# naturerobots/mesh_navigation

Hardware: AMD Instinct MI355X
Metric: plans/sec (Dijkstra makePlan device path incl. computeVectorMap, 1M-vertex mesh) (higher is better)
Workload: dtype f32

## Files before the change

mesh_navigation_amd/csrc/mnav_options.h:

```cpp
#pragma once

#define MNAV_OPTION_LIST(X)                                                                                                              \
  X(verbose)                                                              \
  X(trace)                                                                                       \
  X(no_graph)             \
  X(debug_chunk)                                                                            \
  X(dijkstra_engine)                                 \
  X(blocks_per_plan)                                                                                 \
  X(tile_blocks)                                                                                    \
  X(cvp_wide)                                        \
  X(wide_waves)                                                                                      \
  X(cvp_groups)                          \
  X(max_steps) X(max_wall_s)                                                                                                             \
  X(cvp_verify)                                                                     \
  X(key_walk_max) X(descend_walk_max)                                                               \
  X(tile_size)                                                                                   \
  X(lazy_paths)                                                                                      \
  X(tile_band) X(rounds_band_mult)                                                                                                       \
  X(tb_tile)                                                       \
  X(tb_no_prefill) X(tb_band_mult) X(tb_waves_per_cu)                                                                                    \
  X(tb_kernel)            \
  X(async_wg_per_cu) X(async_wg_per_plan) X(async_max_s)                                                                                 \
  X(async_band_mult)                              \
  X(async_max_batch)                                           \
  X(async_ring_cap)             \
  X(nbhd_lds_cap)         \
  X(replan_log_cap)                                          \
  X(replan_fresh_below)   \
  X(replan_each_fresh_share)  \
  X(replan_repair_engine)  \
  X(replan_warm_min_plans)  \
  X(fleet_scratch_mb)     \
  X(dispatch_max_mb)      \
  X(dispatch_max_rounds)  \
  X(dispatch_tail_bidders)

struct Options {
#define X(name) double name = NAN;
  MNAV_OPTION_LIST(X)
#undef X
  struct Desc { const char* name; double Options::*field; };
  static const Desc* table(size_t* n)
  {
    static const Desc t[] = {
#define X(name) { #name, &Options::name },
      MNAV_OPTION_LIST(X)
#undef X
    };
    *n = sizeof(t) / sizeof(t[0]);
    return t;
  }
  double* find(const char* name)
  {
    size_t n; const Desc* t = table(&n);
    for (size_t i = 0; i < n; ++i) if (!strcmp(t[i].name, name)) return &(this->*t[i].field);
    return nullptr;
  }
  void from_environment()
  {
    size_t n; const Desc* t = table(&n);
    for (size_t i = 0; i < n; ++i) {
      std::string var = "MNAV_";
      for (const char* c = t[i].name; *c; ++c) var += (char)toupper((unsigned char)*c);
      const char* e = getenv(var.c_str());
      if (!e || !*e) continue;
      double v = atof(e);
      if (!strcmp(t[i].name, "dijkstra_engine")) {
        v = !strcmp(e, "tiled") ? 0 : !strcmp(e, "band") ? 1 : !strcmp(e, "tile_batch") ? 5 : !strcmp(e, "async") ? 6
          : (e[0] >= '0' && e[0] <= '9') ? atof(e) : 3;
      }
      this->*t[i].field = v;
    }
  }
};
static inline bool opt_set(double v) { return v == v; }
static inline uint32_t opt_u32(double v, uint32_t dflt) { return v == v ? (uint32_t)(v < 0.0 ? 0.0 : v) : dflt; }
static inline bool opt_on(double v) { return v == v && v != 0.0; }
```

mesh_navigation_amd/csrc/mnav_tb.h:

```cpp
#pragma once

#include "mnav_tb_build.h"

namespace {

namespace tb {

#define MNAV_CONST __attribute__((address_space(4)))
typedef uint32_t u32x16 __attribute__((ext_vector_type(16)));
typedef const MNAV_CONST u32x16* cblk8_t;
typedef __attribute__((address_space(3))) uint32_t* lds_u32_t;
enum { kTwSoff = 0, kTwSl = 1, kTwNv = 2, kTwNh = 3, kTwSweepOff = 4, kTwSweepChunks = 5, kTwPreOff = 6, kTwPreChunks = 7,
       kTwPostOff = 8, kTwPostChunks = 9, kTwExpOff = 10, kTwExpN = 11 };
static_assert(offsetof(TbTile, exp_n) == 4 * kTwExpN && offsetof(TbTile, sweep_off) == 4 * kTwSweepOff, "TbTile layout");

struct Ctl {
  uint32_t n_cand[2];
  uint32_t n_items, next_item;
  uint32_t err;
  uint32_t iters;
  unsigned long long acts;
  unsigned long long sweeps;
  unsigned long long items;
  unsigned long long wakes;
};

struct Args {
  const TbTile* tiles; const uint32_t* stream; const TbExp* exps;
  float* D; uint32_t* pend; uint32_t NP, ntiles;
  uint16_t* bucket; uint32_t* bcnt; uint2* items; Ctl* ctl;
  uint32_t* marr[2];
  uint32_t* mcarry;
  float* thr; float* bnd;
  const uint32_t* seed; const uint32_t* target;
  const uint2* vaddr; const uint32_t* vert_tile;
  double offset; float band;
  uint8_t* pflag; uint32_t nblk;
  unsigned long long* wstat; uint32_t wstat_slots;
  uint32_t item_plans;
};

__device__ __forceinline__ size_t slot_addr(const uint2 va, uint32_t NP, uint32_t p)
{
  return (size_t)va.x * NP + (size_t)p * (va.y >> 8) + (va.y & 255u);
}

__device__ __forceinline__ uint32_t ldsr(uint32_t off) { return *(lds_u32_t)(uintptr_t)off; }
__device__ __forceinline__ void ldsw(uint32_t off, uint32_t v) { *(lds_u32_t)(uintptr_t)off = v; }
typedef __attribute__((address_space(3))) u32x4* lds_u32x4_t;
__device__ __forceinline__ u32x4 ldsr4(uint32_t off) { return *(lds_u32x4_t)(uintptr_t)off; }

__device__ __forceinline__ uint32_t rfl(uint32_t x) { return (uint32_t)__builtin_amdgcn_readfirstlane((int)x); }

}

__global__ __launch_bounds__(kBlock) void k_tb_weights(size_t n, const uint32_t* __restrict__ wsrc, const Nbr* __restrict__ nbr, uint32_t* __restrict__ stream)
{
  const size_t stride = (size_t)gridDim.x * kBlock;
  for (size_t i = (size_t)blockIdx.x * kBlock + threadIdx.x; i < n; i += stride) {
    const uint32_t s = wsrc[i];
    if (s != kNone) stream[i] = f2u(nbr[s].w);
  }
}

__global__ __launch_bounds__(kBlock) void k_tb_fill(u32x4* __restrict__ p, size_t n16, uint32_t v)
{
  const size_t stride = (size_t)gridDim.x * kBlock;
  const u32x4 x = { v, v, v, v };
  for (size_t i = (size_t)blockIdx.x * kBlock + threadIdx.x; i < n16; i += stride) __builtin_nontemporal_store(x, p + i);
}

__global__ __launch_bounds__(kBlock) void k_tb_seed(tb::Args A)
{
  const uint32_t p = blockIdx.x * kBlock + threadIdx.x;
  if (p >= A.NP) return;
  const uint32_t s = A.seed[p];
  const uint2 va = A.vaddr[s];
  A.D[tb::slot_addr(va, A.NP, p)] = 0.0f;
  const uint32_t t = A.vert_tile[s];
  const TbTile W = A.tiles[t];
  const uint32_t row = (va.y & 255u) * 256u;
  for (uint32_t k = 0; k < W.exp_n; ++k) {
    const TbExp e = A.exps[W.exp_off + k];
    if (e.u == row) A.D[(size_t)e.soff * A.NP + (size_t)p * e.sl + e.off] = 0.0f;
  }
  A.pend[(size_t)t * A.NP + p] = 0u;
  A.pflag[(size_t)t * A.nblk + (p >> 6)] = 1;
  A.marr[0][p] = 0u;
  A.ctl->n_cand[0] = 1u;
}

constexpr uint32_t kTbMinCopies = 64;
__global__ __launch_bounds__(kBlock) void k_tb_plan(tb::Args A, int par)
{
  const uint32_t p = blockIdx.x * kBlock + threadIdx.x;
  if (p == 0) { A.ctl->n_cand[par ^ 1] = 0u; A.ctl->next_item = 0u; A.ctl->n_items = 0u; A.ctl->iters += 1u; }
  if (p >= A.NP) return;
  uint32_t mb = A.marr[par][p];
  A.marr[par ^ 1][p] = kTbInfBits;
  {
    uint32_t x[kTbMinCopies];
#pragma unroll
    for (uint32_t c = 0; c < kTbMinCopies; ++c) x[c] = A.mcarry[(size_t)c * A.NP + p];
#pragma unroll
    for (uint32_t c = 0; c < kTbMinCopies; ++c) {
      mb = min(mb, x[c]);
      if (x[c] != kTbInfBits) A.mcarry[(size_t)c * A.NP + p] = kTbInfBits;
    }
  }
  const float m = u2f(mb);
  const float dt = A.D[tb::slot_addr(A.vaddr[A.target[p]], A.NP, p)];
  const float bound = (float)((double)dt + fmax(A.offset, 0.0));
  const bool done = !(m < inf_f()) || m > bound;
  float thr = m + A.band;
  if (!(thr > m)) thr = next_up(m);
  A.thr[p] = done ? 0.0f : thr;
  A.bnd[p] = bound;
}

constexpr uint32_t kTbStatSlots = 16384;
constexpr uint32_t kTbSchedTiles = kBlock / 64;
#ifndef MNAV_TB_SCHED_DEPTH
#define MNAV_TB_SCHED_DEPTH 4
#endif
constexpr uint32_t kTbSchedDepth = MNAV_TB_SCHED_DEPTH;
__global__ __launch_bounds__(kBlock) void k_tb_sched(tb::Args A, int par)
{
  const uint32_t lane = threadIdx.x & 63u;
  const uint32_t t = tb::rfl(blockIdx.x * kTbSchedTiles + (threadIdx.x >> 6));
  if (t >= A.ntiles) return;
  const uint32_t nblk = A.nblk, NP = A.NP;
  MNAV_GLOBAL uint8_t* const g_flag = as_global(A.pflag) + (size_t)t * nblk;
  auto flags = [&](uint32_t c) { const uint32_t i = c * 64u + lane; return i < nblk ? (uint32_t)g_flag[i] : 0u; };
  const uint32_t f0 = flags(0u), f1 = flags(1u);
  unsigned long long m = __ballot(f0 != 0u), m_next = __ballot(f1 != 0u);
  uint32_t c = 0;
  auto next_block = [&]() -> uint32_t {
    while (m == 0ull) {
      if ((c + 1u) * 64u >= nblk) return kNone;
      ++c; m = m_next; m_next = __ballot(flags(c + 1u) != 0u);
    }
    const uint32_t b = c * 64u + (uint32_t)__builtin_ctzll(m);
    m &= m - 1ull;
    return b;
  };
  const uint32_t b_first = next_block();
  if (b_first == kNone) return;
  MNAV_GLOBAL const float* const g_thr = as_global(A.thr);
  MNAV_GLOBAL const float* const g_bnd = as_global(A.bnd);
  MNAV_GLOBAL uint32_t* const g_pend = as_global(A.pend) + (size_t)t * NP;
  MNAV_GLOBAL uint16_t* const g_bucket = as_global(A.bucket) + (size_t)t * NP;
  MNAV_GLOBAL uint32_t* const g_min = as_global(A.mcarry) + (size_t)(t % kTbMinCopies) * NP;
  struct Row { uint32_t p, pb, pm; float thr, bnd; bool live; };
  auto fetch = [&](uint32_t b) {
    Row r;
    const uint32_t p = (b != kNone ? b : 0u) * 64u + lane;
    r.live = b != kNone && p < NP;
    r.p = r.live ? p : 0u;
    r.pb = g_pend[r.p]; r.thr = g_thr[r.p]; r.bnd = g_bnd[r.p]; r.pm = g_min[r.p];
    return r;
  };
  const unsigned long long below = (1ull << lane) - 1ull;
  uint32_t count = 0;
  bool carried = false;
  constexpr int K = (int)kTbSchedDepth;
  uint32_t b_cur[K];
  Row cur[K];
  b_cur[0] = b_first;
#pragma unroll
  for (int k = 1; k < K; ++k) b_cur[k] = next_block();
#pragma unroll
  for (int k = 0; k < K; ++k) cur[k] = fetch(b_cur[k]);
  for (;;) {
    uint32_t b_next[K];
    Row nxt[K];
#pragma unroll
    for (int k = 0; k < K; ++k) b_next[k] = next_block();
#pragma unroll
    for (int k = 0; k < K; ++k) nxt[k] = fetch(b_next[k]);
    __builtin_amdgcn_sched_barrier(0);
#pragma unroll
    for (int k = 0; k < K; ++k)
      asm volatile("" :: "v"(cur[k].pb), "v"(cur[k].thr), "v"(cur[k].bnd), "v"(cur[k].pm));
#pragma unroll
    for (int k = 0; k < K; ++k) {
      if (b_cur[k] == kNone) break;
      const uint32_t p = cur[k].p, pb = cur[k].pb;
      bool ready = false, keep = false;
      if (cur[k].live && pb != kTbInfBits) {
        const float pv = u2f(pb);
        if (pv > cur[k].bnd) g_pend[p] = kTbInfBits;
        else if (pv < cur[k].thr) { g_pend[p] = kTbInfBits; ready = true; }
        else {
          keep = true;
          if (pb < cur[k].pm) atomicMin((uint32_t*)(g_min + p), pb);
        }
      }
      const bool any_keep = __any(keep);
      carried |= any_keep;
      if (!any_keep && lane == 0u) g_flag[b_cur[k]] = 0;
      const unsigned long long rm = __ballot(ready);
      if (ready) g_bucket[count + (uint32_t)__popcll(rm & below)] = (uint16_t)p;
      count += (uint32_t)__popcll(rm);
    }
    if (b_next[0] == kNone) break;
#pragma unroll
    for (int k = 0; k < K; ++k) { cur[k] = nxt[k]; b_cur[k] = b_next[k]; }
  }
  if (lane == 0u) {
    if (count) A.bcnt[t] = count;
    if (carried) A.ctl->n_cand[par ^ 1] = 1u;
  }
}

constexpr uint32_t kTbItemPlans = 16;
__global__ __launch_bounds__(kBlock) void k_tb_items(tb::Args A)
{
  const uint32_t t = blockIdx.x * kBlock + threadIdx.x;
  const int lane = threadIdx.x & 63;
  const uint32_t gran = A.item_plans;
  uint32_t c = 0;
  if (t < A.ntiles) { c = A.bcnt[t]; if (c) A.bcnt[t] = 0u; }
  const uint32_t k = (c + gran - 1u) / gran;
  uint32_t incl = k;
#pragma unroll
  for (int o = 1; o < 64; o <<= 1) { const uint32_t x = __shfl_up(incl, o); if (lane >= o) incl += x; }
  __shared__ uint32_t s_wave[kBlock / 64], s_base;
  const int wave = threadIdx.x >> 6;
  if (lane == 63) s_wave[wave] = incl;
  __syncthreads();
  if (threadIdx.x == 0) {
    uint32_t tot = 0;
#pragma unroll
    for (int w = 0; w < kBlock / 64; ++w) { const uint32_t x = s_wave[w]; s_wave[w] = tot; tot += x; }
    s_base = tot ? atomicAdd(&A.ctl->n_items, tot) : 0u;
  }
  __syncthreads();
  const uint32_t base = s_base + s_wave[wave] + incl - k;
  for (uint32_t q = 0; q < k; ++q) A.items[base + q] = make_uint2(t, (q * gran) | (min(gran, c - q * gran) << 16));
}

__global__ __launch_bounds__(1024) void k_tb_stats(tb::Args A)
{
  __shared__ unsigned long long s_part[16][4];
  unsigned long long acc[4] = { 0ull, 0ull, 0ull, 0ull };
  for (uint32_t w = threadIdx.x; w < A.wstat_slots; w += 1024u)
#pragma unroll
    for (int k = 0; k < 4; ++k) acc[k] += A.wstat[4u * w + k];
#pragma unroll
  for (int k = 0; k < 4; ++k)
#pragma unroll
    for (int o = 32; o > 0; o >>= 1) acc[k] += __shfl_xor(acc[k], o);
  if ((threadIdx.x & 63u) == 0u)
#pragma unroll
    for (int k = 0; k < 4; ++k) s_part[threadIdx.x >> 6][k] = acc[k];
  __syncthreads();
  if (threadIdx.x == 0) {
    unsigned long long t[4] = { 0ull, 0ull, 0ull, 0ull };
    for (int w = 0; w < 16; ++w)
      for (int k = 0; k < 4; ++k) t[k] += s_part[w][k];
    A.ctl->items = t[0]; A.ctl->acts = t[1]; A.ctl->sweeps = t[2]; A.ctl->wakes = t[3];
  }
}

struct TbBlk { uint32_t ya, raw, v[7]; };

#ifdef MNAV_TB_TIMING
__device__ unsigned long long g_tb_timing[8];
#define TB_STAMP(k) do { const unsigned long long now_ = __builtin_readcyclecounter(); tt[k] += now_ - t_last; t_last = now_; } while (0)
#else
#define TB_STAMP(k) do { } while (0)
#endif

constexpr uint32_t kTbQStride = 272;

namespace tb {
__device__ __forceinline__ void ldsw4(uint32_t off, u32x4 v) { *(lds_u32x4_t)(uintptr_t)off = v; }
__device__ __forceinline__ uint32_t wmax4(uint32_t x)
{
  x = max(x, (uint32_t)__shfl_xor((int)x, 16));
  x = max(x, (uint32_t)__shfl_xor((int)x, 32));
  return rfl(x);
}
struct QStream {
  MNAV_GLOBAL const u32x4* st;
  uint32_t last, wr, c; u32x4 c1;
  __device__ __forceinline__ void begin_at(MNAV_GLOBAL const u32x4* first, uint32_t nch, uint32_t stage_q, uint32_t l16)
  {
    st = first + l16;
    last = nch ? nch - 1u : 0u; wr = stage_q + 16u * l16; c = 0;
    ldsw4(wr, st[0]);
    c1 = st[(size_t)min(1u, last) * 16u];
  }
  __device__ __forceinline__ void begin(MNAV_GLOBAL const uint32_t* stream, uint32_t chunk_off, uint32_t nch, uint32_t stage_q, uint32_t l16)
  {
    begin_at((MNAV_GLOBAL const u32x4*)(stream + (size_t)chunk_off * kTbChunk), nch, stage_q, l16);
  }
  __device__ __forceinline__ void advance()
// ... 387 lines not shown
    const uint32_t beg = row_ptr[v], end = row_ptr[v + 1];
    for (uint32_t i = beg + lane; i < end; i += kWave) {
      const Nbr nb = nbr[i];
      const float du = A.D[tb::slot_addr(A.vaddr[nb.u], A.NP, p)];
      if (!expanded_source(gcut, du, nb.u)) continue;
      const float sm = du + nb.w;
      if (sm < best_s || (sm == best_s && sm < inf_f() && (du < best_du || (du == best_du && nb.u < best_u)))) { best_s = sm; best_du = du; best_u = nb.u; }
    }
#pragma unroll
    for (int o = 1; o < kWave; o <<= 1) {
      const float os = __shfl_xor(best_s, o), odu = __shfl_xor(best_du, o);
      const uint32_t ou = __shfl_xor(best_u, o);
      if (os < best_s || (os == best_s && os < inf_f() && (odu < best_du || (odu == best_du && ou < best_u)))) { best_s = os; best_du = odu; best_u = ou; }
    }
    if (!(best_s < inf_f())) best_u = v;
  }
  if (lane == 0) {
    float x = 0.f, y = 0.f, z = 0.f;
    if (best_u != v) {
      x = xyz[3 * (size_t)best_u] - xyz[3 * (size_t)v];
      y = xyz[3 * (size_t)best_u + 1] - xyz[3 * (size_t)v + 1];
      z = xyz[3 * (size_t)best_u + 2] - xyz[3 * (size_t)v + 2];
      const float len = sqrtf(x * x + y * y + z * z);
      x = x / len; y = y / len; z = z / len;
    }
    out[3 * blockIdx.x] = x; out[3 * blockIdx.x + 1] = y; out[3 * blockIdx.x + 2] = z;
  }
}

__global__ __launch_bounds__(kBlock) void k_tb_count(tb::Args A, uint32_t T, PlanResult* __restrict__ res)
{
  const uint32_t t = blockIdx.x;
  const int lane = threadIdx.x & 63, wid = threadIdx.x >> 6;
  const TbTile W = A.tiles[t];
  for (uint32_t p = blockIdx.y * (kBlock / 64) + wid; p < A.NP; p += gridDim.y * (kBlock / 64)) {
    const float dt = A.D[tb::slot_addr(A.vaddr[A.target[p]], A.NP, p)];
    const float goal_dist = goal_cut(dt, A.offset, A.target[p]).cut;
    const float* sl = A.D + ((size_t)W.soff * A.NP + (size_t)p * W.sl);
    uint32_t c = 0;
    for (uint32_t i = lane; i < W.nv; i += 64) { const float d = sl[i]; c += (d < inf_f() && d <= goal_dist) ? 1u : 0u; }
    c = wave_sum(c);
    if (lane == 0 && c) atomicAdd(&res[p].settled, (unsigned long long)c);
  }
}

__global__ __launch_bounds__(kBlock) void k_tb_popped(tb::Args A, uint32_t p, uint32_t V, float* __restrict__ out)
{
  const float dt = A.D[tb::slot_addr(A.vaddr[A.target[p]], A.NP, p)];
  const float goal_dist = goal_cut(dt, A.offset, A.target[p]).cut;
  const uint32_t stride = gridDim.x * kBlock;
  for (uint32_t v = blockIdx.x * kBlock + threadIdx.x; v < V; v += stride) {
    const float d = A.D[tb::slot_addr(A.vaddr[v], A.NP, p)];
    out[v] = (d <= goal_dist) ? d : inf_f();
  }
}

__global__ __launch_bounds__(kBlock) void k_popped(const float* __restrict__ dist, uint32_t target, double offset, uint32_t V, float* __restrict__ out)
{
  const float dt = dist[target];
  const float goal_dist = goal_cut(dt, offset, target).cut;
  const uint32_t stride = gridDim.x * kBlock;
  for (uint32_t v = blockIdx.x * kBlock + threadIdx.x; v < V; v += stride) { const float d = dist[v]; out[v] = (d <= goal_dist) ? d : inf_f(); }
}

struct TbTables {
  bool built = false, w_valid = false;
  uint32_t ntiles = 0, max_nh = 0;
  uint64_t S = 0;
  size_t nrec = 0, nexp = 0;
  std::vector<uint32_t> vert_tile;
  DevBuf<uint32_t> d_verts;
  DevBuf<TbTile> d_tiles; DevBuf<uint32_t> d_stream, d_wsrc; DevBuf<TbExp> d_exps;
  DevBuf<uint32_t> d_vstream, d_vwsrc, d_vtile, d_vgroups; DevBuf<TbvExp> d_vexps; size_t nvrec = 0;
  DevBuf<uint2> d_vaddr; DevBuf<uint32_t> d_vert_tile;
  DevBuf<uint16_t> d_fin_src; DevBuf<uint32_t> d_fin_wsrc; DevBuf<float> d_fin_w; DevBuf<TbFinOvf> d_fin_ovf; DevBuf<uint32_t> d_fin_ovf_wsrc; DevBuf<float> d_fin_ovf_w;
  DevBuf<uint32_t> d_ghost_gid, d_fin_order; size_t fin_n = 0, fin_novf = 0; bool fin_w_valid = false; uint32_t max_sl = 0;
};

struct TbBatch {
  uint32_t cap_np = 0;
  DevBuf<float> D; DevBuf<uint32_t> pend; DevBuf<uint32_t> mcarry; DevBuf<uint8_t> pflag; DevBuf<uint16_t> bucket; DevBuf<uint32_t> bcnt; DevBuf<uint2> items;
  DevBuf<tb::Ctl> ctl; PinnedBuf<tb::Ctl> h_ctl;
  DevBuf<unsigned long long> wstat; DevBuf<struct FinRec> d_recs;
  DevBuf<uint32_t> marr[2];
  DevBuf<float> thr, bnd; DevBuf<uint32_t> seed, target;
  GraphExec graph[2]; tb::Args graph_args[2]{};
  DevBuf<float> D2; bool d2_clean = false; uint32_t d2_clean_np = 0, d2_wanted_np = 0;
};

struct TbState : TbTables, TbBatch {
  uint32_t T = 120;
  int kernel = 0;
  uint32_t min_batch = 48;
  float band_mult = 2.0f;
  int iters_per_replay = 16, waves_per_cu = 0;
  Stream fill_stream; Event fill_done, call_done;
  Event warm_ev[4]; float ms_warm = 0.f, ms_warm_fin = 0.f;
  tb::Ctl last{};
  bool count_pending = false;
};

}

#ifdef MNAV_TB_TIMING
extern "C" int mnav_debug_tb_timing(unsigned long long* out)
{
  if (hipMemcpyFromSymbol(out, HIP_SYMBOL(g_tb_timing), sizeof(unsigned long long) * 8) != hipSuccess) return -1;
  unsigned long long z[8] = { 0, 0, 0, 0, 0, 0, 0, 0 };
  return hipMemcpyToSymbol(HIP_SYMBOL(g_tb_timing), z, sizeof(z)) == hipSuccess ? 0 : -1;
}
#endif
```

mesh_navigation_amd/csrc/mnav_tb_host.h:

```cpp
#pragma once

void tb_free_batch(mnav_ctx* ctx)
{
  TbState& S = ctx->tb;
  if (S.fill_stream) (void)hipStreamSynchronize(S.fill_stream);
  static_cast<TbBatch&>(S) = TbBatch{};
  S.count_pending = false; ctx->tb_args_valid = false;
}

void tb_free(mnav_ctx* ctx)
{
  tb_free_batch(ctx);
  static_cast<TbTables&>(ctx->tb) = TbTables{};
}

int tb_build(mnav_ctx* ctx)
{
  TbState& S = ctx->tb;
  if (S.built) return 0;
  if (opt_set(ctx->opt.tb_tile)) S.T = opt_u32(ctx->opt.tb_tile, S.T);
  if (S.T != 64 && S.T != 96 && S.T != 120 && S.T != 128) S.T = 120;
  HostTopology t;
  t.V = ctx->V; t.E = ctx->E; t.F = ctx->F;
  t.row_ptr = ctx->h_row_ptr; t.nbr_u = ctx->h_nbr_u;
// ... 19 lines not shown
  HIPCHK(S.d_vaddr.upload(ctx->stream, vaddr.data(), vaddr.size()));
  HIPCHK(S.d_vert_tile.upload(ctx->stream, H.vert_tile.data(), H.vert_tile.size()));
  HIPCHK(S.d_verts.upload(ctx->stream, H.verts.data(), H.verts.size()));
  HIPCHK(S.d_fin_src.upload(ctx->stream, H.fin_src.data(), H.fin_src.size()));
  HIPCHK(S.d_fin_wsrc.upload(ctx->stream, H.fin_wsrc.data(), H.fin_wsrc.size()));
  HIPCHK(S.d_fin_ovf.upload(ctx->stream, H.fin_ovf.data(), H.fin_ovf.size()));
  {
    std::vector<uint32_t> ow(H.fin_ovf.size());
    for (size_t i = 0; i < ow.size(); ++i) ow[i] = H.fin_ovf[i].wsrc;
    HIPCHK(S.d_fin_ovf_wsrc.upload(ctx->stream, ow.data(), ow.size()));
  }
  HIPCHK(S.d_ghost_gid.upload(ctx->stream, H.ghost_gid.data(), H.ghost_gid.size()));
  {
    std::vector<uint32_t> order(H.tiles.size()), key(H.tiles.size(), 0xFFFFFFFFu);
    for (size_t t = 0; t < H.tiles.size(); ++t) {
      order[t] = (uint32_t)t;
      for (uint32_t i = 0; i < H.tiles[t].nv; ++i) key[t] = std::min(key[t], H.verts[H.tiles[t].v0 + i]);
    }
    std::stable_sort(order.begin(), order.end(), [&](uint32_t a, uint32_t b) { return key[a] < key[b]; });
    if (order.empty()) order.push_back(0u);
    HIPCHK(S.d_fin_order.upload(ctx->stream, order.data(), order.size()));
  }
  S.d_fin_w.reset(); S.d_fin_ovf_w.reset();
  S.fin_n = H.fin_src.size(); S.fin_novf = H.fin_ovf.size(); S.fin_w_valid = false; S.max_sl = H.max_sl;
  HIPCHK(S.d_fin_w.alloc(4 * std::max<size_t>(S.fin_n, 1)));
  HIPCHK(S.d_fin_ovf_w.alloc(4 * std::max<size_t>(S.fin_novf, 1)));
  HIPCHK(hipStreamSynchronize(ctx->stream));
  S.nvrec = H.vstream.size();
  S.ntiles = H.ntiles; S.S = H.S; S.nrec = H.stream.size(); S.nexp = H.exps.size(); S.max_nh = H.max_nh;
  S.vert_tile = std::move(H.vert_tile);
  S.built = true; S.w_valid = false;
  if (opt_on(ctx->opt.verbose))
    fprintf(stderr, "[mnav] tile-batch engine: T %u, %u tiles, %.2f slots per vertex, max ghosts %u, %.1f MB of streams + %.1f MB of sweep streams in the V layout\n", S.T, S.ntiles,
            ctx->V ? (double)S.S / ctx->V : 0.0, S.max_nh, (4.0 * S.nrec + 16.0 * S.nexp) / 1e6, 4.0 * S.nvrec / 1e6);
  return 0;
}

int tb_weights(mnav_ctx* ctx)
{
  TbState& S = ctx->tb;
  if (S.w_valid) return 0;
  hipLaunchKernelGGL(k_tb_weights, dim3(4096), dim3(kBlock), 0, ctx->stream, S.nrec, S.d_wsrc, ctx->d_nbr, S.d_stream);
  hipLaunchKernelGGL(k_tb_weights, dim3(4096), dim3(kBlock), 0, ctx->stream, S.nvrec, S.d_vwsrc, ctx->d_nbr, S.d_vstream);
  HIPCHK(hipGetLastError());
  S.w_valid = true; S.fin_w_valid = false;
  return 0;
}

int tb_fin_weights(mnav_ctx* ctx)
{
  TbState& S = ctx->tb;
  if (S.fin_w_valid) return 0;
  hipLaunchKernelGGL(k_tb_fin_weights, dim3(4096), dim3(kBlock), 0, ctx->stream, S.fin_n, S.d_fin_wsrc, ctx->d_nbr, S.d_fin_w);
  if (S.fin_novf) hipLaunchKernelGGL(k_tb_fin_weights, dim3(64), dim3(kBlock), 0, ctx->stream, S.fin_novf, S.d_fin_ovf_wsrc, ctx->d_nbr, S.d_fin_ovf_w);
  HIPCHK(hipGetLastError());
  S.fin_w_valid = true;
  return 0;
}

int tb_ensure_batch(mnav_ctx* ctx, uint32_t np)
{
  TbState& S = ctx->tb;
  if (np <= S.cap_np) return 0;
  tb_free_batch(ctx);
  const size_t nt = S.ntiles ? S.ntiles : 1, pairs = nt * (size_t)np;
  HIPCHK(S.D.alloc(4 * (size_t)S.S * np + 64));
  if (8 * (size_t)S.S * np <= ((size_t)96 << 30) && !opt_on(ctx->opt.tb_no_prefill)) {
    if (S.D2.alloc(4 * (size_t)S.S * np + 64) != hipSuccess) (void)hipGetLastError();
    if (S.D2 && !S.fill_stream) { HIPCHK(hipStreamCreateWithFlags(S.fill_stream.out(), hipStreamNonBlocking)); HIPCHK(hipEventCreateWithFlags(S.fill_done.out(), hipEventDisableTiming)); HIPCHK(hipEventCreateWithFlags(S.call_done.out(), hipEventDisableTiming)); }
  }
  HIPCHK(S.pend.alloc(4 * pairs + 64));
  HIPCHK(S.pflag.alloc(nt * (((size_t)np + 63) / 64) + 64));
  HIPCHK(S.bucket.alloc(2 * pairs + 64));
  HIPCHK(S.bcnt.alloc(4 * nt));
  HIPCHK(S.items.alloc(8 * (nt + pairs / kTbItemPlans + 64)));
  HIPCHK(S.ctl.alloc(sizeof(tb::Ctl)));
  HIPCHK(S.wstat.alloc(32 * (size_t)kTbStatSlots));
  HIPCHK(S.h_ctl.alloc(sizeof(tb::Ctl)));
  for (int k = 0; k < 2; ++k) HIPCHK(S.marr[k].alloc(4 * (size_t)np));
  HIPCHK(S.mcarry.alloc(4 * (size_t)kTbMinCopies * np + 64));
  HIPCHK(S.thr.alloc(4 * (size_t)np)); HIPCHK(S.bnd.alloc(4 * (size_t)np));
  HIPCHK(S.seed.alloc(4 * (size_t)np)); HIPCHK(S.target.alloc(4 * (size_t)np));
  HIPCHK(S.d_recs.alloc(sizeof(FinRec) * (size_t)np));
  S.cap_np = np;
  return 0;
}

int tb_fill(mnav_ctx* ctx, void* p, size_t bytes, uint32_t v)
{
  const size_t n16 = (bytes + 15) / 16;
  uint32_t g = (uint32_t)std::min<size_t>((n16 + kBlock - 1) / kBlock, 256 * 32);
  if (g < 1) g = 1;
  hipLaunchKernelGGL(k_tb_fill, dim3(g), dim3(kBlock), 0, ctx->stream, (u32x4*)p, n16, v);
  HIPCHK(hipGetLastError());
  return 0;
}

int tb_launch_iterations(mnav_ctx* ctx, const tb::Args& A, int count, uint32_t waves)
{
  const uint32_t gp = (A.NP + kBlock - 1) / kBlock;
  for (int j = 0; j < count; ++j) {
    const int par = j & 1;
    hipLaunchKernelGGL(k_tb_plan, dim3(gp), dim3(kBlock), 0, ctx->stream, A, par);
    hipLaunchKernelGGL(k_tb_sched, dim3(std::max((A.ntiles + kTbSchedTiles - 1) / kTbSchedTiles, 1u)), dim3(kBlock), 0, ctx->stream, A, par);
    hipLaunchKernelGGL(k_tb_items, dim3((A.ntiles + kBlock - 1) / kBlock), dim3(kBlock), 0, ctx->stream, A);
    if (ctx->tb.kernel == 1) hipLaunchKernelGGL((k_tbv_solve<120>), dim3(waves), dim3(64), 0, ctx->stream, A, ctx->tb.d_vtile, ctx->tb.d_vstream, ctx->tb.d_vgroups, ctx->tb.d_vexps, par);
    else if (ctx->tb.T == 64) hipLaunchKernelGGL((k_tb_solve_q<64>), dim3(waves), dim3(64), 0, ctx->stream, A, par);
    else if (ctx->tb.T == 96) hipLaunchKernelGGL((k_tb_solve_q<96>), dim3(waves), dim3(64), 0, ctx->stream, A, par);
    else if (ctx->tb.T == 120) hipLaunchKernelGGL((k_tb_solve_q<120>), dim3(waves), dim3(64), 0, ctx->stream, A, par);
    else hipLaunchKernelGGL((k_tb_solve_q<128>), dim3(waves), dim3(64), 0, ctx->stream, A, par);
  }
  hipLaunchKernelGGL(k_tb_stats, dim3(1), dim3(1024), 0, ctx->stream, A);
  HIPCHK(hipGetLastError());
  return 0;
}

int tb_fields(mnav_ctx* ctx, uint32_t n, const std::vector<PlanIn>& in, double offset, const tb::Args& A)
{
  TbState& S = ctx->tb;
  if (ensure_slots(ctx, n, false, false, ctx->want_vec)) return -1;
  if (tb_fin_weights(ctx)) return -1;
  std::vector<Plan> hp(n);
  std::vector<float*> vecs(n);
  for (uint32_t i = 0; i < n; ++i) {
    Slot& s = ctx->slots[i];
    Plan& P = hp[i];
    memset(&P, 0, sizeof(P));
    P.planner = kPlannerDijkstra; P.V = ctx->V;
    P.row_ptr = ctx->d_row_ptr.get(); P.nbr = ctx->d_nbr.get(); P.crn_ptr = ctx->d_crn_ptr.get(); P.crn = ctx->d_crn.get(); P.blocked = ctx->d_blocked.get();
    P.dist = s.dist.get(); P.pred = s.pred.get(); P.cap = ctx->V; P.ctl = s.ctl; P.cnt = s.cnt.get();
    P.offset = offset; P.max_steps = ctx->max_steps;
    for (int k = 0; k < 3; ++k) { P.seed[k] = in[i].seed[k]; P.target[k] = in[i].target[k]; P.seed_d[k] = 0.f; P.seed_expands[k] = 1; P.target_expands[k] = 1; }
    P.seed_face = kNone;
    vecs[i] = s.vecmap;
  }
  HIPCHK(hipMemcpyAsync(ctx->d_plans, hp.data(), sizeof(Plan) * n, hipMemcpyHostToDevice, ctx->stream));
  HIPCHK(hipMemcpyAsync(ctx->d_vecptrs, vecs.data(), sizeof(float*) * n, hipMemcpyHostToDevice, ctx->stream));
  HIPCHK(hipStreamSynchronize(ctx->stream));
  FinTb F{};
  F.src = S.d_fin_src; F.w = S.d_fin_w; F.ovf = S.d_fin_ovf; F.ovf_w = S.d_fin_ovf_w; F.verts = S.d_verts; F.ghost_gid = S.d_ghost_gid; F.order = S.d_fin_order;
  F.xyz = ctx->d_xyz; F.vecmaps = ctx->want_vec ? ctx->d_vecptrs : nullptr;
  F.plans = ctx->d_plans; F.res = ctx->d_res; F.mismatch = ctx->d_mismatch; F.recs = S.d_recs;
  const uint32_t groups = (S.ntiles + kFinWaves - 1u) / kFinWaves;
#ifndef MNAV_FIN_PPW
#define MNAV_FIN_PPW 64u
#endif
  F.plans_per_wave = MNAV_FIN_PPW; F.tiles_per_xcd = (groups + 7u) / 8u; F.max_sl = S.max_sl;
  hipLaunchKernelGGL(k_tb_fin_plans, dim3((n + kBlock - 1) / kBlock), dim3(kBlock), 0, ctx->stream, A, ctx->d_plans, F.vecmaps, S.d_recs);
  const uint32_t npg = (n + F.plans_per_wave - 1u) / F.plans_per_wave;
  const size_t lds = 4 * (size_t)fin_lds_words(S.max_sl, F.vecmaps != nullptr) * kFinWaves;
  const dim3 grid(8u * F.tiles_per_xcd * npg);
  if (S.T == 64) hipLaunchKernelGGL((k_tb_finalize<64>), grid, dim3(64 * kFinWaves), lds, ctx->stream, A, F);
  else if (S.T == 96) hipLaunchKernelGGL((k_tb_finalize<96>), grid, dim3(64 * kFinWaves), lds, ctx->stream, A, F);
  else if (S.T == 120) hipLaunchKernelGGL((k_tb_finalize<120>), grid, dim3(64 * kFinWaves), lds, ctx->stream, A, F);
  else hipLaunchKernelGGL((k_tb_finalize<128>), grid, dim3(64 * kFinWaves), lds, ctx->stream, A, F);
  HIPCHK(hipGetLastError());
  return 0;
}

int tb_clean_other(mnav_ctx* ctx)
{
  TbState& S = ctx->tb;
  if (!S.D2 || !S.fill_stream || S.d2_wanted_np == 0u || S.d2_clean) return 0;
  const uint32_t n = S.d2_wanted_np;
  S.d2_wanted_np = 0u;
  const size_t n16 = (4 * (size_t)S.S * n + 15) / 16;
  const uint32_t g = (uint32_t)std::max<size_t>(std::min<size_t>((n16 + kBlock - 1) / kBlock, 256 * 32), 1);
  HIPCHK(hipEventRecord(S.call_done, ctx->stream));
  HIPCHK(hipStreamWaitEvent(S.fill_stream, S.call_done, 0));
  hipLaunchKernelGGL(k_tb_fill, dim3(g), dim3(kBlock), 0, S.fill_stream, (u32x4*)S.D2.get(), n16, kTbInfBits);
  HIPCHK(hipEventRecord(S.fill_done, S.fill_stream));
  S.d2_clean = true; S.d2_clean_np = n;
  return 0;
}

struct TbWarmIn { const uint32_t* d_level; const float* const* d_dist; ReplanCnt* d_cnt; };

int run_dijkstra_tb(mnav_ctx* ctx, uint32_t n, const std::vector<PlanIn>& in, double offset, const TbWarmIn* warm = nullptr)
{
  TbState& S = ctx->tb;
  if (tb_build(ctx)) return -1;
  if (tb_weights(ctx)) return -1;
  if (n > 65535u) { ctx->err = "tile-batch engine: more than 65535 plans in one batch"; return -1; }
  if (tb_ensure_batch(ctx, n)) return -1;
  if (ensure_plan_tables(ctx, n)) return -1;
  if (ensure_paths(ctx, n)) return -1;
  if (!ctx->d_mismatch) HIPCHK(ctx->d_mismatch.alloc(4));
  std::vector<uint32_t> seeds(n), targets(n);
  for (uint32_t i = 0; i < n; ++i) { seeds[i] = in[i].seed[0]; targets[i] = in[i].target[0]; }
  HIPCHK(hipMemcpyAsync(S.seed, seeds.data(), 4 * (size_t)n, hipMemcpyHostToDevice, ctx->stream));
  HIPCHK(hipMemcpyAsync(S.target, targets.data(), 4 * (size_t)n, hipMemcpyHostToDevice, ctx->stream));
  HIPCHK(hipMemsetAsync(ctx->d_res, 0, sizeof(PlanResult) * n, ctx->stream));
  HIPCHK(hipMemsetAsync(ctx->d_mismatch, 0, 4, ctx->stream));
  tb::Args A{};
  A.tiles = S.d_tiles; A.stream = S.d_stream; A.exps = S.d_exps; A.D = S.D; A.pend = S.pend; A.pflag = S.pflag; A.nblk = (n + 63u) / 64u; A.NP = n; A.ntiles = S.ntiles;
  A.bucket = S.bucket; A.bcnt = S.bcnt; A.items = S.items; A.ctl = S.ctl; A.wstat = S.wstat; A.wstat_slots = kTbStatSlots;
  A.marr[0] = S.marr[0]; A.marr[1] = S.marr[1]; A.mcarry = S.mcarry;
  A.thr = S.thr; A.bnd = S.bnd; A.seed = S.seed; A.target = S.target; A.vaddr = S.d_vaddr; A.vert_tile = S.d_vert_tile;
  A.offset = offset;
  const bool v_fits = S.T == 120 && S.max_nh <= kTbvGhostRows;
  const double density = (double)n / std::sqrt((double)std::max(S.ntiles, 1u));
  S.kernel = (v_fits && density >= 8.0) ? 1 : 0;
  if (opt_set(ctx->opt.tb_kernel)) S.kernel = (opt_u32(ctx->opt.tb_kernel, 0u) == 1u && v_fits) ? 1 : 0;
  A.item_plans = S.kernel == 1 ? 64u : kTbItemPlans;
  {
    const float band_mult = (S.kernel == 1 && density < 40.0) ? 4.0f : S.band_mult;
    float band = (ctx->delta_auto / 3.0f) * std::sqrt((float)S.T) * band_mult;
    if (opt_set(ctx->opt.tb_band_mult)) band = (ctx->delta_auto / 3.0f) * std::sqrt((float)S.T) * (float)ctx->opt.tb_band_mult;
    if (ctx->tile_band_user > 0.f) band = ctx->tile_band_user;
    A.band = band;
  }
  HIPCHK(hipEventRecord(ctx->ev[1], ctx->stream));
  if (!warm) {
    bool prefilled = false;
    if (S.D2 && S.d2_clean && S.d2_clean_np >= n) {
      std::swap(S.D, S.D2); A.D = S.D;
      HIPCHK(hipStreamWaitEvent(ctx->stream, S.fill_done, 0));
      prefilled = true;
    }
    S.d2_clean = false;
    if (!prefilled && tb_fill(ctx, S.D, 4 * (size_t)S.S * n, kTbInfBits)) return -1;
    if (tb_fill(ctx, S.pend, 4 * (size_t)S.ntiles * n, kTbInfBits)) return -1;
  }
  HIPCHK(hipMemsetAsync(S.pflag, 0, (size_t)(S.ntiles ? S.ntiles : 1) * ((n + 63u) / 64u) + 64u, ctx->stream));
  if (tb_fill(ctx, S.marr[0], 4 * (size_t)n, kTbInfBits)) return -1;
  if (tb_fill(ctx, S.marr[1], 4 * (size_t)n, kTbInfBits)) return -1;
  if (tb_fill(ctx, S.mcarry, 4 * (size_t)kTbMinCopies * n, kTbInfBits)) return -1;
  HIPCHK(hipMemsetAsync(S.ctl, 0, sizeof(tb::Ctl), ctx->stream));
  HIPCHK(hipMemsetAsync(S.wstat, 0, 32 * (size_t)kTbStatSlots, ctx->stream));
  HIPCHK(hipMemsetAsync(S.bcnt, 0, 4 * (size_t)(S.ntiles ? S.ntiles : 1), ctx->stream));
  if (warm) {
    if (!S.warm_ev[0]) for (auto& e : S.warm_ev) HIPCHK(hipEventCreate(e.out()));
    HIPCHK(hipMemsetAsync(warm->d_cnt, 0, sizeof(ReplanCnt) * (size_t)n, ctx->stream));
    TbWarm Wm{};
    Wm.level = warm->d_level; Wm.dist = warm->d_dist; Wm.cnt = warm->d_cnt;
    Wm.verts = S.d_verts; Wm.ghost_gid = S.d_ghost_gid; Wm.order = S.d_fin_order; Wm.T = S.T;
    const size_t groups = (size_t)std::max(S.ntiles, 1u) * ((n + 63u) / 64u);
    if (groups >= (1ull << 31)) { ctx->err = "tile-batch engine: warm start beyond 2^31 workgroups"; return -1; }
    HIPCHK(hipEventRecord(S.warm_ev[0], ctx->stream));
    if (S.ntiles) hipLaunchKernelGGL(k_tb_warm, dim3((uint32_t)groups), dim3(kWarmBlock), 0, ctx->stream, A, Wm);
    HIPCHK(hipEventRecord(S.warm_ev[1], ctx->stream));
  } else
  hipLaunchKernelGGL(k_tb_seed, dim3((n + kBlock - 1) / kBlock), dim3(kBlock), 0, ctx->stream, A);
  HIPCHK(hipGetLastError());
  HIPCHK(hipEventRecord(ctx->ev[2], ctx->stream));
  if (!warm || !S.d2_clean) S.d2_wanted_np = S.D2 ? n : 0u;

  int ncu = 256;
  (void)hipDeviceGetAttribute(&ncu, hipDeviceAttributeMultiprocessorCount, ctx->device);
  uint32_t per_cu = (uint32_t)((160u * 1024u) / (S.T * 256u + kTbQStride * 4u));
  if (S.kernel == 1) per_cu = 8u;
  if (opt_set(ctx->opt.tb_waves_per_cu)) S.waves_per_cu = (int)ctx->opt.tb_waves_per_cu;
  if (S.waves_per_cu > 0) per_cu = (uint32_t)S.waves_per_cu;
  const uint32_t waves = std::min(per_cu * (uint32_t)ncu, kTbStatSlots);
  const int chunk = S.iters_per_replay & ~1;
  int gi = 0;
  for (int k = 0; k < 2; ++k) if (S.graph[k] && memcmp(&S.graph_args[k], &A, sizeof(A)) == 0) gi = k + 2;
  if (ctx->use_graph && gi < 2) {
    gi = (S.graph[0] && S.graph_args[0].D != A.D) ? 1 : 0;
    S.graph[gi].reset();
    hipGraph_t g = nullptr;
    HIPCHK(hipStreamBeginCapture(ctx->stream, hipStreamCaptureModeThreadLocal));
    const int rc = tb_launch_iterations(ctx, A, chunk, waves);
    const hipError_t e = hipStreamEndCapture(ctx->stream, &g);
    if (rc != 0 || e != hipSuccess) { ctx->err = "graph capture failed"; return -1; }
    HIPCHK(hipGraphInstantiate(S.graph[gi].out(), g, nullptr, nullptr, 0));
    (void)hipGraphDestroy(g);
    memcpy(&S.graph_args[gi], &A, sizeof(A));
  } else gi -= 2;
  int rc = 0;
  uint32_t iters = 0;
  const auto t_start = std::chrono::steady_clock::now();
  HIPCHK(hipEventRecord(ctx->evc[0], ctx->stream));
  for (;;) {
    if (std::chrono::duration<double>(std::chrono::steady_clock::now() - t_start).count() > ctx->max_wall_s) {
      ctx->err = "tile-batch iterations exceeded the wall-clock guard"; return -1;
    }
    if (ctx->use_graph) HIPCHK(hipGraphLaunch(S.graph[gi], ctx->stream));
    else if (tb_launch_iterations(ctx, A, chunk, waves)) return -1;
    iters += (uint32_t)chunk;
    HIPCHK(hipMemcpyAsync(S.h_ctl, S.ctl, sizeof(tb::Ctl), hipMemcpyDeviceToHost, ctx->stream));
    HIPCHK(hipStreamSynchronize(ctx->stream));
    if (S.h_ctl->err) { ctx->err = "tile-batch engine: sweep cap hit"; return -1; }
    if (S.h_ctl->n_cand[0] == 0u) break;
    if (ctx->cancel.load(std::memory_order_relaxed)) { rc = 1; break; }
    if (iters > ctx->max_steps) { ctx->err = "tile-batch engine: iteration cap hit"; return -1; }
  }
  HIPCHK(hipEventRecord(ctx->evc[1], ctx->stream));
  if (rc == 0 && !ctx->lazy_paths) {
    if (warm) HIPCHK(hipEventRecord(S.warm_ev[2], ctx->stream));
    if (tb_fields(ctx, n, in, offset, A)) return -1;
    if (warm) HIPCHK(hipEventRecord(S.warm_ev[3], ctx->stream));
  }
  HIPCHK(hipEventRecord(ctx->ev[3], ctx->stream));
  HIPCHK(hipEventSynchronize(ctx->evc[1]));
  ctx->ms_chunks = ev_ms(ctx->evc[0], ctx->evc[1]);
  S.last = *S.h_ctl;
  if (warm && rc == 0) {
    HIPCHK(hipEventSynchronize(S.warm_ev[3]));
    S.ms_warm = ev_ms(S.warm_ev[0], S.warm_ev[1]); S.ms_warm_fin = ev_ms(S.warm_ev[2], S.warm_ev[3]);
  }
  ctx->stats.launches = 1;
  ctx->tb_args = A; ctx->tb_args_valid = (rc == 0);
  if (opt_on(ctx->opt.trace))
    fprintf(stderr, "[mnav] tile-batch: %u iterations, %llu activations (%.1f per item), %llu items, %.2f sweeps per item, %llu wakes\n", S.h_ctl->iters,
            S.h_ctl->acts, S.h_ctl->items ? (double)S.h_ctl->acts / S.h_ctl->items : 0.0, S.h_ctl->items,
            S.h_ctl->items ? (double)S.h_ctl->sweeps / S.h_ctl->items : 0.0, S.h_ctl->wakes);
  return rc;
}
```

Before: 43270.

## Reduce carried per-plan minima in LDS and overlap field-setup upload

The scheduler kernel now uses 16 waves per workgroup and accumulates per-plan carried minima in LDS when the plan count fits in 64 KiB. The block flushes them to a few global copies only when something was carried. The plan kernel then reads 4 copies instead of 64, which cuts global atomics and per-iteration reads. Separately, the host-side plan and vecmap upload for computeVectorMap moves before the iteration loop into pinned buffers, dropping a stream synchronize. The cost is LDS initialization per workgroup and larger blocks with lower occupancy.

```diff
diff --git a/mesh_navigation_amd/csrc/mnav_options.h b/mesh_navigation_amd/csrc/mnav_options.h
--- a/mesh_navigation_amd/csrc/mnav_options.h
+++ b/mesh_navigation_amd/csrc/mnav_options.h
@@ -20,7 +20,8 @@
   X(tb_tile)                                                       \
   X(tb_no_prefill) X(tb_band_mult) X(tb_waves_per_cu)                                                                                    \
   X(tb_kernel)            \
-  X(async_wg_per_cu) X(async_wg_per_plan) X(async_max_s)                                                                                 \
+  X(tb_sched_lds)         \
+  X(async_wg_per_cu) X(async_wg_per_plan) X(async_max_s)                                                                              \
   X(async_band_mult)                              \
   X(async_max_batch)                                           \
   X(async_ring_cap)             \
diff --git a/mesh_navigation_amd/csrc/mnav_tb.h b/mesh_navigation_amd/csrc/mnav_tb.h
--- a/mesh_navigation_amd/csrc/mnav_tb.h
+++ b/mesh_navigation_amd/csrc/mnav_tb.h
@@ -38,6 +38,7 @@
   uint8_t* pflag; uint32_t nblk;
   unsigned long long* wstat; uint32_t wstat_slots;
   uint32_t item_plans;
+  uint32_t sched_lds, min_copies;
 };
 
 __device__ __forceinline__ size_t slot_addr(const uint2 va, uint32_t NP, uint32_t p)
@@ -91,6 +92,12 @@
 }
 
 constexpr uint32_t kTbMinCopies = 64;
+#ifndef MNAV_TB_MIN_COPIES_LDS
+#define MNAV_TB_MIN_COPIES_LDS 4
+#endif
+constexpr uint32_t kTbMinCopiesLds = MNAV_TB_MIN_COPIES_LDS;
+static_assert(kTbMinCopiesLds >= 1 && kTbMinCopiesLds <= kTbMinCopies, "the LDS path's copies are the first ones of mcarry");
+template <uint32_t NC>
 __global__ __launch_bounds__(kBlock) void k_tb_plan(tb::Args A, int par)
 {
   const uint32_t p = blockIdx.x * kBlock + threadIdx.x;
@@ -99,11 +106,11 @@
   uint32_t mb = A.marr[par][p];
   A.marr[par ^ 1][p] = kTbInfBits;
   {
-    uint32_t x[kTbMinCopies];
-#pragma unroll
-    for (uint32_t c = 0; c < kTbMinCopies; ++c) x[c] = A.mcarry[(size_t)c * A.NP + p];
-#pragma unroll
-    for (uint32_t c = 0; c < kTbMinCopies; ++c) {
+    uint32_t x[NC];
+#pragma unroll
+    for (uint32_t c = 0; c < NC; ++c) x[c] = A.mcarry[(size_t)c * A.NP + p];
+#pragma unroll
+    for (uint32_t c = 0; c < NC; ++c) {
       mb = min(mb, x[c]);
       if (x[c] != kTbInfBits) A.mcarry[(size_t)c * A.NP + p] = kTbInfBits;
     }
@@ -119,16 +126,25 @@
 }
 
 constexpr uint32_t kTbStatSlots = 16384;
-constexpr uint32_t kTbSchedTiles = kBlock / 64;
+#ifndef MNAV_TB_SCHED_TILES
+#define MNAV_TB_SCHED_TILES 16
+#endif
+constexpr uint32_t kTbSchedTiles = MNAV_TB_SCHED_TILES;
+static_assert(kTbSchedTiles >= 1 && kTbSchedTiles <= 16, "a workgroup holds at most 16 waves");
+constexpr uint32_t kTbSchedLdsMax = 64u * 1024u;
+inline bool tb_sched_lds_fits(uint32_t np) { return 4u * ((size_t)np + 1u) <= kTbSchedLdsMax; }
+#ifndef MNAV_TB_SCHED_FLUSH
+#define MNAV_TB_SCHED_FLUSH 8
+#endif
+constexpr uint32_t kTbSchedFlush = MNAV_TB_SCHED_FLUSH;
 #ifndef MNAV_TB_SCHED_DEPTH
 #define MNAV_TB_SCHED_DEPTH 4
 #endif
 constexpr uint32_t kTbSchedDepth = MNAV_TB_SCHED_DEPTH;
-__global__ __launch_bounds__(kBlock) void k_tb_sched(tb::Args A, int par)
-{
-  const uint32_t lane = threadIdx.x & 63u;
-  const uint32_t t = tb::rfl(blockIdx.x * kTbSchedTiles + (threadIdx.x >> 6));
-  if (t >= A.ntiles) return;
+template <bool LDS>
+__device__ __forceinline__ void tb_sched_walk(const tb::Args& A, uint32_t t, uint32_t lane, MNAV_GLOBAL uint32_t* g_min, uint32_t* s_min,
+                                              uint32_t& count, bool& carried)
+{
   const uint32_t nblk = A.nblk, NP = A.NP;
   MNAV_GLOBAL uint8_t* const g_flag = as_global(A.pflag) + (size_t)t * nblk;
   auto flags = [&](uint32_t c) { const uint32_t i = c * 64u + lane; return i < nblk ? (uint32_t)g_flag[i] : 0u; };
@@ -150,19 +166,17 @@
   MNAV_GLOBAL const float* const g_bnd = as_global(A.bnd);
   MNAV_GLOBAL uint32_t* const g_pend = as_global(A.pend) + (size_t)t * NP;
   MNAV_GLOBAL uint16_t* const g_bucket = as_global(A.bucket) + (size_t)t * NP;
-  MNAV_GLOBAL uint32_t* const g_min = as_global(A.mcarry) + (size_t)(t % kTbMinCopies) * NP;
   struct Row { uint32_t p, pb, pm; float thr, bnd; bool live; };
   auto fetch = [&](uint32_t b) {
     Row r;
     const uint32_t p = (b != kNone ? b : 0u) * 64u + lane;
     r.live = b != kNone && p < NP;
     r.p = r.live ? p : 0u;
-    r.pb = g_pend[r.p]; r.thr = g_thr[r.p]; r.bnd = g_bnd[r.p]; r.pm = g_min[r.p];
+    r.pb = g_pend[r.p]; r.thr = g_thr[r.p]; r.bnd = g_bnd[r.p];
+    r.pm = LDS ? 0u : g_min[r.p];
     return r;
   };
   const unsigned long long below = (1ull << lane) - 1ull;
-  uint32_t count = 0;
-  bool carried = false;
   constexpr int K = (int)kTbSchedDepth;
   uint32_t b_cur[K];
   Row cur[K];
@@ -180,8 +194,10 @@
     for (int k = 0; k < K; ++k) nxt[k] = fetch(b_next[k]);
     __builtin_amdgcn_sched_barrier(0);
 #pragma unroll
-    for (int k = 0; k < K; ++k)
-      asm volatile("" :: "v"(cur[k].pb), "v"(cur[k].thr), "v"(cur[k].bnd), "v"(cur[k].pm));
+    for (int k = 0; k < K; ++k) {
+      asm volatile("" :: "v"(cur[k].pb), "v"(cur[k].thr), "v"(cur[k].bnd));
+      if (!LDS) asm volatile("" :: "v"(cur[k].pm));
+    }
 #pragma unroll
     for (int k = 0; k < K; ++k) {
       if (b_cur[k] == kNone) break;
@@ -193,7 +209,8 @@
         else if (pv < cur[k].thr) { g_pend[p] = kTbInfBits; ready = true; }
         else {
           keep = true;
-          if (pb < cur[k].pm) atomicMin((uint32_t*)(g_min + p), pb);
+          if (LDS) atomicMin(s_min + p, pb);
+          else if (pb < cur[k].pm) atomicMin((uint32_t*)(g_min + p), pb);
         }
       }
       const bool any_keep = __any(keep);
@@ -207,13 +224,49 @@
 #pragma unroll
     for (int k = 0; k < K; ++k) { cur[k] = nxt[k]; b_cur[k] = b_next[k]; }
   }
+}
+
+constexpr uint32_t kTbItemPlans = 16;
+
+template <bool LDS>
+__global__ __launch_bounds__(kTbSchedTiles * 64) void k_tb_sched(tb::Args A, int par)
+{
+  constexpr uint32_t G = kTbSchedTiles, kThreads = G * 64u;
+  extern __shared__ uint32_t s_dyn[];
+  uint32_t* const s_carried = s_dyn; uint32_t* const s_min = s_dyn + 1u;
+  const uint32_t lane = threadIdx.x & 63u, wave = tb::rfl(threadIdx.x >> 6);
+  const uint32_t t = blockIdx.x * G + wave, NP = A.NP;
+  if (LDS) {
+    for (uint32_t i = threadIdx.x; i < NP; i += kThreads) s_min[i] = kTbInfBits;
+    if (threadIdx.x == 0u) *s_carried = 0u;
+    __syncthreads();
+  }
+  MNAV_GLOBAL uint32_t* const g_min = as_global(A.mcarry) + (size_t)(LDS ? blockIdx.x % kTbMinCopiesLds : t % kTbMinCopies) * NP;
+  uint32_t count = 0;
+  bool carried = false;
+  if (t < A.ntiles) tb_sched_walk<LDS>(A, t, lane, g_min, s_min, count, carried);
   if (lane == 0u) {
     if (count) A.bcnt[t] = count;
-    if (carried) A.ctl->n_cand[par ^ 1] = 1u;
-  }
-}
-
-constexpr uint32_t kTbItemPlans = 16;
+    if (carried) {
+      if (LDS) *s_carried = 1u;
+      A.ctl->n_cand[par ^ 1] = 1u;
+    }
+  }
+  if (!LDS) return;
+  __syncthreads();
+  if (*s_carried == 0u) return;
+  constexpr uint32_t kU = kTbSchedFlush;
+  for (uint32_t i0 = threadIdx.x; i0 < NP; i0 += kU * kThreads) {
+    uint32_t v[kU], pm[kU];
+#pragma unroll
+    for (uint32_t j = 0; j < kU; ++j) { const uint32_t i = i0 + j * kThreads; v[j] = i < NP ? s_min[i] : kTbInfBits; }
+#pragma unroll
+    for (uint32_t j = 0; j < kU; ++j) pm[j] = v[j] != kTbInfBits ? g_min[i0 + j * kThreads] : 0u;
+#pragma unroll
+    for (uint32_t j = 0; j < kU; ++j) if (v[j] < pm[j]) atomicMin((uint32_t*)(g_min + (i0 + j * kThreads)), v[j]);
+  }
+}
+
 __global__ __launch_bounds__(kBlock) void k_tb_items(tb::Args A)
 {
   const uint32_t t = blockIdx.x * kBlock + threadIdx.x;
@@ -767,6 +820,7 @@
   DevBuf<float> D; DevBuf<uint32_t> pend; DevBuf<uint32_t> mcarry; DevBuf<uint8_t> pflag; DevBuf<uint16_t> bucket; DevBuf<uint32_t> bcnt; DevBuf<uint2> items;
   DevBuf<tb::Ctl> ctl; PinnedBuf<tb::Ctl> h_ctl;
   DevBuf<unsigned long long> wstat; DevBuf<struct FinRec> d_recs;
+  PinnedBuf<Plan> h_plans; PinnedBuf<float*> h_vecs;
   DevBuf<uint32_t> marr[2];
   DevBuf<float> thr, bnd; DevBuf<uint32_t> seed, target;
   GraphExec graph[2]; tb::Args graph_args[2]{};
diff --git a/mesh_navigation_amd/csrc/mnav_tb_host.h b/mesh_navigation_amd/csrc/mnav_tb_host.h
--- a/mesh_navigation_amd/csrc/mnav_tb_host.h
+++ b/mesh_navigation_amd/csrc/mnav_tb_host.h
@@ -125,6 +125,7 @@
   HIPCHK(S.thr.alloc(4 * (size_t)np)); HIPCHK(S.bnd.alloc(4 * (size_t)np));
   HIPCHK(S.seed.alloc(4 * (size_t)np)); HIPCHK(S.target.alloc(4 * (size_t)np));
   HIPCHK(S.d_recs.alloc(sizeof(FinRec) * (size_t)np));
+  HIPCHK(S.h_plans.alloc(sizeof(Plan) * (size_t)np)); HIPCHK(S.h_vecs.alloc(sizeof(float*) * (size_t)np));
   S.cap_np = np;
   return 0;
 }
@@ -142,10 +143,17 @@
 int tb_launch_iterations(mnav_ctx* ctx, const tb::Args& A, int count, uint32_t waves)
 {
   const uint32_t gp = (A.NP + kBlock - 1) / kBlock;
+  const dim3 gs(std::max((A.ntiles + kTbSchedTiles - 1) / kTbSchedTiles, 1u)), bs(kTbSchedTiles * 64u);
+  const size_t lds_s = A.sched_lds ? 4 * ((size_t)A.NP + 1u) : 0;
   for (int j = 0; j < count; ++j) {
     const int par = j & 1;
-    hipLaunchKernelGGL(k_tb_plan, dim3(gp), dim3(kBlock), 0, ctx->stream, A, par);
-    hipLaunchKernelGGL(k_tb_sched, dim3(std::max((A.ntiles + kTbSchedTiles - 1) / kTbSchedTiles, 1u)), dim3(kBlock), 0, ctx->stream, A, par);
+    if (A.sched_lds) {
+      hipLaunchKernelGGL((k_tb_plan<kTbMinCopiesLds>), dim3(gp), dim3(kBlock), 0, ctx->stream, A, par);
+      hipLaunchKernelGGL((k_tb_sched<true>), gs, bs, lds_s, ctx->stream, A, par);
+    } else {
+      hipLaunchKernelGGL((k_tb_plan<kTbMinCopies>), dim3(gp), dim3(kBlock), 0, ctx->stream, A, par);
+      hipLaunchKernelGGL((k_tb_sched<false>), gs, bs, lds_s, ctx->stream, A, par);
+    }
     hipLaunchKernelGGL(k_tb_items, dim3((A.ntiles + kBlock - 1) / kBlock), dim3(kBlock), 0, ctx->stream, A);
     if (ctx->tb.kernel == 1) hipLaunchKernelGGL((k_tbv_solve<120>), dim3(waves), dim3(64), 0, ctx->stream, A, ctx->tb.d_vtile, ctx->tb.d_vstream, ctx->tb.d_vgroups, ctx->tb.d_vexps, par);
     else if (ctx->tb.T == 64) hipLaunchKernelGGL((k_tb_solve_q<64>), dim3(waves), dim3(64), 0, ctx->stream, A, par);
@@ -158,13 +166,13 @@
   return 0;
 }
 
-int tb_fields(mnav_ctx* ctx, uint32_t n, const std::vector<PlanIn>& in, double offset, const tb::Args& A)
+int tb_fields_upload(mnav_ctx* ctx, uint32_t n, const std::vector<PlanIn>& in, double offset)
 {
   TbState& S = ctx->tb;
   if (ensure_slots(ctx, n, false, false, ctx->want_vec)) return -1;
   if (tb_fin_weights(ctx)) return -1;
-  std::vector<Plan> hp(n);
-  std::vector<float*> vecs(n);
+  Plan* const hp = S.h_plans.get();
+  float** const vecs = S.h_vecs.get();
   for (uint32_t i = 0; i < n; ++i) {
     Slot& s = ctx->slots[i];
     Plan& P = hp[i];
@@ -177,9 +185,14 @@
     P.seed_face = kNone;
     vecs[i] = s.vecmap;
   }
-  HIPCHK(hipMemcpyAsync(ctx->d_plans, hp.data(), sizeof(Plan) * n, hipMemcpyHostToDevice, ctx->stream));
-  HIPCHK(hipMemcpyAsync(ctx->d_vecptrs, vecs.data(), sizeof(float*) * n, hipMemcpyHostToDevice, ctx->stream));
-  HIPCHK(hipStreamSynchronize(ctx->stream));
+  HIPCHK(hipMemcpyAsync(ctx->d_plans, hp, sizeof(Plan) * n, hipMemcpyHostToDevice, ctx->stream));
+  HIPCHK(hipMemcpyAsync(ctx->d_vecptrs, vecs, sizeof(float*) * n, hipMemcpyHostToDevice, ctx->stream));
+  return 0;
+}
+
+int tb_fields(mnav_ctx* ctx, uint32_t n, const tb::Args& A)
+{
+  TbState& S = ctx->tb;
   FinTb F{};
   F.src = S.d_fin_src; F.w = S.d_fin_w; F.ovf = S.d_fin_ovf; F.ovf_w = S.d_fin_ovf_w; F.verts = S.d_verts; F.ghost_gid = S.d_ghost_gid; F.order = S.d_fin_order;
   F.xyz = ctx->d_xyz; F.vecmaps = ctx->want_vec ? ctx->d_vecptrs : nullptr;
@@ -235,6 +248,7 @@
   HIPCHK(hipMemcpyAsync(S.target, targets.data(), 4 * (size_t)n, hipMemcpyHostToDevice, ctx->stream));
   HIPCHK(hipMemsetAsync(ctx->d_res, 0, sizeof(PlanResult) * n, ctx->stream));
   HIPCHK(hipMemsetAsync(ctx->d_mismatch, 0, 4, ctx->stream));
+  if (!ctx->lazy_paths && tb_fields_upload(ctx, n, in, offset)) return -1;
   tb::Args A{};
   A.tiles = S.d_tiles; A.stream = S.d_stream; A.exps = S.d_exps; A.D = S.D; A.pend = S.pend; A.pflag = S.pflag; A.nblk = (n + 63u) / 64u; A.NP = n; A.ntiles = S.ntiles;
   A.bucket = S.bucket; A.bcnt = S.bcnt; A.items = S.items; A.ctl = S.ctl; A.wstat = S.wstat; A.wstat_slots = kTbStatSlots;
@@ -246,6 +260,8 @@
   S.kernel = (v_fits && density >= 8.0) ? 1 : 0;
   if (opt_set(ctx->opt.tb_kernel)) S.kernel = (opt_u32(ctx->opt.tb_kernel, 0u) == 1u && v_fits) ? 1 : 0;
   A.item_plans = S.kernel == 1 ? 64u : kTbItemPlans;
+  A.sched_lds = (tb_sched_lds_fits(n) && !(opt_set(ctx->opt.tb_sched_lds) && !opt_on(ctx->opt.tb_sched_lds))) ? 1u : 0u;
+  A.min_copies = A.sched_lds ? kTbMinCopiesLds : kTbMinCopies;
   {
     const float band_mult = (S.kernel == 1 && density < 40.0) ? 4.0f : S.band_mult;
     float band = (ctx->delta_auto / 3.0f) * std::sqrt((float)S.T) * band_mult;
@@ -332,7 +348,7 @@
   HIPCHK(hipEventRecord(ctx->evc[1], ctx->stream));
   if (rc == 0 && !ctx->lazy_paths) {
     if (warm) HIPCHK(hipEventRecord(S.warm_ev[2], ctx->stream));
-    if (tb_fields(ctx, n, in, offset, A)) return -1;
+    if (tb_fields(ctx, n, A)) return -1;
     if (warm) HIPCHK(hipEventRecord(S.warm_ev[3], ctx->stream));
   }
   HIPCHK(hipEventRecord(ctx->ev[3], ctx->stream));
@@ -346,8 +362,8 @@
   ctx->stats.launches = 1;
   ctx->tb_args = A; ctx->tb_args_valid = (rc == 0);
   if (opt_on(ctx->opt.trace))
-    fprintf(stderr, "[mnav] tile-batch: %u iterations, %llu activations (%.1f per item), %llu items, %.2f sweeps per item, %llu wakes\n", S.h_ctl->iters,
+    fprintf(stderr, "[mnav] tile-batch: %u iterations, %llu activations (%.1f per item), %llu items, %.2f sweeps per item, %llu wakes, carried minima %s\n", S.h_ctl->iters,
             S.h_ctl->acts, S.h_ctl->items ? (double)S.h_ctl->acts / S.h_ctl->items : 0.0, S.h_ctl->items,
-            S.h_ctl->items ? (double)S.h_ctl->sweeps / S.h_ctl->items : 0.0, S.h_ctl->wakes);
+            S.h_ctl->items ? (double)S.h_ctl->sweeps / S.h_ctl->items : 0.0, S.h_ctl->wakes, A.sched_lds ? "reduced in LDS" : "in global memory");
   return rc;
 }
```

Result: faster. 43820 (median of 6 runs) (+1.3%).
